# MarbleHE/ABC

Hardware: AMD Instinct MI355X
Metric: homomorphic mul+relin/sec, CKKS N=2^14 (higher is better)
Workload: dtype u64 (transforms: exact integer arithmetic in f64); 1 GPU; CKKS N=16384, 4 data limbs {50,40,40,40} + special 50-bit prime, ct x ct multiply + relinearize; total_batch=8192, batch_rank0=8192

## Files before the change

abc_amd/csrc/abc_context.hip:

```cpp
#include <cstdlib>
#include <cstring>
#include <mutex>

#include "../../include/abc_hip.h"
#include <dlfcn.h>

#include "abc_context.hpp"
#include "abc_host_math.hpp"

namespace abc {

static thread_local std::string g_err;
void set_error(const std::string &msg) { g_err = msg; }

static bool env_on(const char *name) {
  const char *e = std::getenv(name);
  return e && !(e[0] == '0' && e[1] == 0);
}
void read_switches(abc_hip_ctx *c) {
  abc_hip_ctx::Switches s;
  s.no_fused = env_on("ABC_HIP_NO_FUSED");
  s.no_split = env_on("ABC_HIP_NO_SPLIT");
  s.no_split4 = env_on("ABC_HIP_NO_SPLIT4");
  s.no_isplit = env_on("ABC_HIP_NO_ISPLIT");
  s.no_gsplit = env_on("ABC_HIP_NO_GSPLIT");
  s.no_bsplit = env_on("ABC_HIP_NO_BSPLIT");
  s.no_mixed = env_on("ABC_HIP_NO_MIXED");
  s.no_pack = env_on("ABC_HIP_NO_PACK");
  s.no_key_twin = env_on("ABC_HIP_NO_KEY_TWIN");
  s.no_bmul = env_on("ABC_HIP_NO_BMUL");
  s.no_iks = env_on("ABC_HIP_NO_IKS");
  s.no_lean_front = env_on("ABC_HIP_NO_LEAN_FRONT");
  s.no_tensor_intt = env_on("ABC_HIP_NO_TENSOR_INTT");
  s.no_galois_fusion = env_on("ABC_HIP_NO_GALOIS_FUSION");
  if (const char *e = std::getenv("ABC_HIP_CHUNK")) s.chunk = (size_t)std::atol(e);
  if (const char *e = std::getenv("ABC_HIP_FEW_LIMBS")) s.few_limbs = (size_t)std::atol(e);
  if (const char *e = std::getenv("ABC_HIP_LEAN_LIMIT")) s.lean_limit = (size_t)std::atol(e);
  if (const char *e = std::getenv("ABC_HIP_PASS0_TARGET_LIMIT")) s.pass0_target_limit = (size_t)std::atol(e);
  if (const char *e = std::getenv("ABC_HIP_BFV_SCRATCH_MB")) s.bfv_scratch_mb = (size_t)std::atol(e);
  if (const char *e = std::getenv("ABC_HIP_LANES")) {
    s.lanes = std::atoi(e);
    if (s.lanes < 1) s.lanes = 1;
    if (s.lanes > abc_hip_ctx::kMaxLanes) s.lanes = abc_hip_ctx::kMaxLanes;
  }
  c->sw = s;
}

static bool capturing(abc_hip_ctx *c) {
  hipStreamCaptureStatus st = hipStreamCaptureStatusNone;
  if (hipStreamIsCapturing(c->stream, &st) != hipSuccess) return false;
  return st != hipStreamCaptureStatusNone;
}

static int trim_cache(abc_hip_ctx *c) {
  std::lock_guard<std::mutex> lock(c->alloc_mu);
  if (c->free_blocks.empty()) return 0;
  ABC_HIP_CHECK(hipStreamSynchronize(c->stream));
  for (auto &kv : c->free_blocks)
    for (void *p : kv.second) {
      c->block_size.erase(p);
      (void)hipFree(p);
    }
  c->free_blocks.clear();
  c->cached_bytes = 0;
  return 0;
}
static hipError_t malloc_retry(abc_hip_ctx *c, void **p, size_t bytes) {
  hipError_t e = hipMalloc(p, bytes);
  if (e == hipSuccess) return e;
  (void)hipGetLastError();
  if (trim_cache(c)) return e;
  return hipMalloc(p, bytes);
}

void retire_buffer(abc_hip_ctx *c, void *p, uint64_t born) {
  if (!p) return;
  abc_hip_ctx::Held h{p, {}};
  for (auto &kv : c->live_graphs)
    if (kv.second > born) h.graphs.push_back(kv.first);
  if (h.graphs.empty()) {
    (void)hipFree(p);
    return;
  }
  c->held.push_back(std::move(h));
}

int ensure_workspace(abc_hip_ctx *c, size_t bytes) {
// ... 481 lines not shown
  }
}

int abc_hip_create_primes(size_t n, const int *bit_sizes, int count, uint64_t *out) {
  try {
    std::map<int, std::vector<uint64_t>> table;
    for (int i = 0; i < count; i++) table[bit_sizes[i]];
    for (auto &kv : table) {
      size_t need = 0;
      for (int i = 0; i < count; i++) need += (bit_sizes[i] == kv.first);
      kv.second = host::ntt_primes(n, kv.first, need);
    }
    for (int i = 0; i < count; i++) {
      auto &v = table[bit_sizes[i]];
      out[i] = v.back();
      v.pop_back();
    }
    return 0;
  } catch (const std::exception &e) {
    set_error(e.what());
    return 1;
  }
}

int abc_hip_ctx_create(int scheme, int logn, const uint64_t *primes, int nprimes, uint64_t plain_modulus, int device,
                       abc_hip_ctx **out) {
  if (!out) { set_error("null output pointer"); return 1; }
  *out = nullptr;
  if (scheme != ABC_HIP_SCHEME_BFV && scheme != ABC_HIP_SCHEME_CKKS) { set_error("unknown scheme"); return 1; }
  if (logn < 10 || logn > 16) { set_error("logn must be in 10..16"); return 1; }
  if (nprimes < 2 || nprimes > kMaxLimbs) { set_error("need 2..16 primes (data limbs + special prime)"); return 1; }
  const uint64_t two_n = 2ull << logn;
  for (int i = 0; i < nprimes; i++) {
    if (primes[i] >> 60 || !host::is_prime(primes[i]) || primes[i] % two_n != 1) {
      set_error("coefficient modulus primes must be < 2^60, prime and = 1 mod 2N");
      return 1;
    }
    for (int j = 0; j < i; j++)
      if (primes[j] == primes[i]) { set_error("coefficient modulus primes must be distinct"); return 1; }
  }
  if (scheme == ABC_HIP_SCHEME_BFV) {
    if (!host::is_prime(plain_modulus) || plain_modulus % two_n != 1 || plain_modulus >> 32) {
      set_error("plain modulus must be a prime = 1 mod 2N (batching) below 2^32");
      return 1;
    }
  }
  int ndev = 0;
  if (hipGetDeviceCount(&ndev) != hipSuccess || ndev <= 0) { set_error("no HIP device available"); return 1; }
  if (device < 0 || device >= ndev) { set_error("device index out of range"); return 1; }
  if (hipSetDevice(device) != hipSuccess) { set_error("hipSetDevice failed"); return 1; }
  abc_hip_ctx *c = new abc_hip_ctx();
  c->scheme = scheme; c->logn = logn; c->n = 1 << logn; c->K = nprimes; c->L = nprimes - 1; c->device = device;
  c->primes.assign(primes, primes + nprimes);
  c->t = (scheme == ABC_HIP_SCHEME_BFV) ? plain_modulus : 0;
  int rc = 1;
  try {
    rc = build_context(c);
  } catch (const std::exception &e) {
    set_error(e.what());
  }
  if (!rc && hipStreamCreateWithFlags(&c->own_stream, hipStreamNonBlocking) != hipSuccess) {
    set_error("hipStreamCreate failed");
    rc = 1;
  }
  if (!rc) c->stream = c->own_stream;
  if (!rc && (hipEventCreate(&c->ev0) != hipSuccess || hipEventCreate(&c->ev1) != hipSuccess ||
              hipEventCreateWithFlags(&c->lane_fork, hipEventDisableTiming) != hipSuccess)) {
    set_error("hipEventCreate failed");
    rc = 1;
  }
  for (int i = 0; !rc && i < abc_hip_ctx::kMaxLanes; i++) {
    if (hipStreamCreateWithFlags(&c->lane[i], hipStreamNonBlocking) != hipSuccess ||
        hipEventCreateWithFlags(&c->lane_join[i], hipEventDisableTiming) != hipSuccess) {
      set_error("lane stream / event creation failed");
      rc = 1;
    }
  }
  if (!rc && !env_on("ABC_HIP_SYNC_ALLOC")) {
    c->cache_alloc = true;
    size_t free_b = 0, total_b = 0;
    if (hipMemGetInfo(&free_b, &total_b) == hipSuccess) c->cache_cap = total_b / 4;
  }
  if (rc) { abc_hip_ctx_destroy(c); return 1; }
  *out = c;
  return 0;
}

void abc_hip_ctx_destroy(abc_hip_ctx *c) {
  if (!c) return;
  (void)hipSetDevice(c->device);
  (void)hipDeviceSynchronize();
  (void)hipFree(c->d_mods); (void)hipFree(c->d_tw); (void)hipFree(c->d_ftw); (void)hipFree(c->d_cst); (void)hipFree(c->d_cstf);
  (void)hipFree(c->d_slot_map);
  (void)hipFree(c->d_ckks_codec);
  drop_key_twins(c, nullptr);
  (void)hipFree(c->d_sk); (void)hipFree(c->d_pk); (void)hipFree(c->d_relin);
  for (auto &kv : c->d_galois) (void)hipFree(kv.second);
  (void)hipFree(c->ws);
  for (void *p : c->aux) (void)hipFree(p);
  for (auto &h : c->held) (void)hipFree(h.p);
  for (auto &kv : c->block_size) (void)hipFree(kv.first);
  if (c->own_stream) (void)hipStreamDestroy(c->own_stream);
  if (c->ev0) (void)hipEventDestroy(c->ev0);
  if (c->ev1) (void)hipEventDestroy(c->ev1);
  if (c->lane_fork) (void)hipEventDestroy(c->lane_fork);
  for (int i = 0; i < abc_hip_ctx::kMaxLanes; i++) {
// ... 487 lines not shown
```

abc_amd/csrc/abc_context.hpp:

```cpp
#pragma once

#include <hip/hip_runtime.h>

#include <map>
#include <mutex>
#include <unordered_map>
#include <string>
#include <vector>

#include "abc_modarith.hpp"
#include "abc_ntt.hpp"

namespace abc {

constexpr int kMaxLimbs = 16;

struct LimbMap {
  int id[kMaxLimbs + 1];
};

struct DevConst {
  u64 inv_special[kMaxLimbs], inv_special_s[kMaxLimbs];
  u64 inv_qlast[kMaxLimbs][kMaxLimbs], inv_qlast_s[kMaxLimbs][kMaxLimbs];
  u64 special_mod_q[kMaxLimbs], special_mod_q_s[kMaxLimbs];
// ... 24 lines not shown
  u64 tgamma_mod_q[kMaxLimbs], q_to_t[kMaxLimbs], q_to_gamma[kMaxLimbs];
  u64 neg_inv_q_mod_t, neg_inv_q_mod_gamma, inv_gamma_mod_t, gamma;
};

struct DevConstFp {
  double ext_q[kMaxLimbs][2], flr_q[kMaxLimbs][2], B_mod_q[kMaxLimbs][2];
  double q_to_bsk[kMaxLimbs][kMaxLimbs][2];
  double B_to_q[kMaxLimbs][kMaxLimbs][2];
  double q_mod_bsk[kMaxLimbs][2], inv_mtilde_mod_bsk[kMaxLimbs][2], tinvq_bsk[kMaxLimbs][2], inv_q_mod_bsk[kMaxLimbs][2];
  double inv_punct_B[kMaxLimbs][2], B_to_msk[kMaxLimbs][2], inv_B_mod_msk[2];
};

struct DevCtx {
  const Mod *mods;
  const u64 *tw;
  const double *ftw;
  const DevConst *cst;
  const DevConstFp *cstf;
  const u32 *slot_map;
  int logn, n;
  int ps;
  int K, L;
  int id_bsk, id_t, id_gamma, id_mtilde;
};

__device__ __forceinline__ NttTable ntt_table(const DevCtx &c, int mid) {
  const u64 *b = c.tw + (size_t)mid * 4 * c.n;
  NttTable t;
  t.tw = reinterpret_cast<const u64x2 *>(b);
  t.itw = reinterpret_cast<const u64x2 *>(b + 2 * (size_t)c.n);
  return t;
}

__device__ __forceinline__ Mod mod_at(const DevCtx &c, int id) {
  const ABC_CONST_AS Mod *p = (const ABC_CONST_AS Mod *)(c.mods + id);
  Mod m;
  m.q = p->q; m.mu = p->mu; m.two_q = p->two_q; m.shift = p->shift; m.bits = p->bits;
  m.inv_n = p->inv_n; m.inv_n_s = p->inv_n_s; m.qd = p->qd; m.qinv = p->qinv;
  m.inv_n_c = p->inv_n_c; m.inv_n_cq = p->inv_n_cq;
  return m;
}
__device__ __forceinline__ FpTable fp_table(const DevCtx &c, int mid) {
  const double *b = c.ftw + (size_t)mid * 4 * c.n;
  FpTable t;
  t.tw = (const ABC_CONST_AS f64x2 *)(b);
  t.itw = (const ABC_CONST_AS f64x2 *)(b + 2 * (size_t)c.n);
  return t;
}

}

struct abc_hip_ctx {
  int scheme = 0, logn = 0, n = 0, K = 0, L = 0, device = 0;
  std::vector<uint64_t> primes;
  uint64_t t = 0;
  hipStream_t stream = nullptr;
  hipStream_t own_stream = nullptr;
  hipEvent_t ev0 = nullptr, ev1 = nullptr;
  static constexpr int kMaxLanes = 4;
  hipStream_t lane[kMaxLanes] = {nullptr, nullptr, nullptr, nullptr};
  hipEvent_t lane_fork = nullptr, lane_join[kMaxLanes] = {nullptr, nullptr, nullptr, nullptr};
  std::vector<abc::Mod> h_mods;
  std::vector<uint64_t> mod_values;
  int nB = 0, nBsk = 0;
  abc::DevCtx dc{};
  abc::DevConst h_cst{};
  abc::Mod *d_mods = nullptr;
  uint64_t *d_tw = nullptr;
  double *d_ftw = nullptr;
  bool cache_alloc = false;
  std::mutex alloc_mu;
  size_t cached_bytes = 0, cache_cap = (size_t)8 << 30;
  std::unordered_map<size_t, std::vector<void *>> free_blocks;
  std::unordered_map<void *, size_t> block_size;
  bool capture_active = false;
  std::unordered_map<void *, std::vector<void *>> pin;
  std::unordered_map<void *, bool> parked;
  std::unordered_map<size_t, std::vector<void *>> cap_free;
  std::unordered_map<void *, bool> cap_born;
  bool behz_fp = false;
  bool use_fp = true;
  struct Switches {
    bool no_fused = false, no_split = false, no_split4 = false, no_isplit = false, no_gsplit = false, no_lean_front = false, no_bsplit = false, no_mixed = false, no_pack = false, no_key_twin = false, no_bmul = false, no_iks = false, no_tensor_intt = false;
    bool no_galois_fusion = false;
    size_t chunk = 0, few_limbs = 48, lean_limit = 96, bfv_scratch_mb = 0, pass0_target_limit = 128;
    int lanes = 2;
  } sw;
  abc::DevConst *d_cst = nullptr;
  abc::DevConstFp *d_cstf = nullptr;
  uint32_t *d_slot_map = nullptr;
  void *d_ckks_codec = nullptr;
  uint64_t *d_sk = nullptr, *d_pk = nullptr, *d_relin = nullptr;
  std::map<uint32_t, uint64_t *> d_galois;
  std::unordered_map<const uint64_t *, double *> key_twins;
  std::unordered_map<const uint64_t *, uint64_t *> key_shoups;
  std::vector<uint32_t> galois_order;
  void *ws = nullptr;
  size_t ws_bytes = 0;
  void *aux[3] = {nullptr, nullptr, nullptr};
  size_t aux_bytes[3] = {0, 0, 0};
  uint64_t graph_seq = 0;
  std::unordered_map<void *, uint64_t> live_graphs;
  struct Held {
    void *p;
    std::vector<void *> graphs;
  };
  std::vector<Held> held;
  uint64_t ws_born = 0, aux_born[3] = {0, 0, 0};
  size_t limb_words() const { return (size_t)n; }
  size_t key_words() const { return (size_t)L * 2 * K * n; }
};

namespace abc {

void set_error(const std::string &msg);
#define ABC_HIP_CHECK(expr)                                                                         \
  do {                                                                                              \
    hipError_t e_ = (expr);                                                                         \
    if (e_ != hipSuccess) {                                                                         \
      abc::set_error(std::string(#expr) + ": " + hipGetErrorString(e_));                            \
      return 1;                                                                                     \
    }                                                                                               \
  } while (0)

int ensure_workspace(abc_hip_ctx *c, size_t bytes);
int ensure_aux(abc_hip_ctx *c, int which, size_t bytes);
void retire_buffer(abc_hip_ctx *c, void *p, uint64_t born);
void read_switches(abc_hip_ctx *c);

LimbMap key_limb_map(const abc_hip_ctx *c, int nl);
int launch_ntt_fwd(abc_hip_ctx *c, u64 *d, const LimbMap &map, int nl, size_t total_limbs);
int launch_ks_expand_ntt_fp(abc_hip_ctx *c, const u64 *tcoef, size_t tstride, u64 *dec, const LimbMap &map, int nl, size_t count);
int launch_ntt_fwd_from2(abc_hip_ctx *c, const u64 *src, const u64 *src2, u64 *d, const LimbMap &map, int nl, size_t total_limbs);
int launch_ntt_fwd_from(abc_hip_ctx *c, const u64 *src, u64 *d, const LimbMap &map, int nl, size_t total_limbs);
int launch_ntt_inv(abc_hip_ctx *c, u64 *d, const LimbMap &map, int nl, size_t total_limbs);
int launch_ntt_inv_strided_part(abc_hip_ctx *c, u64 *d, const LimbMap &map, int nl, size_t total_limbs, bool integer_only = false);
int big_block_log(void);
// ... 146 lines not shown
```

abc_amd/csrc/abc_kernels_fused.hip:

```cpp
#include <type_traits>

#include "abc_context.hpp"
#include "abc_host_math.hpp"

namespace abc {

static inline unsigned stream_grid(size_t items, int block) {
  size_t g = (items + block - 1) / block;
  const size_t cap = 256 * 8 * 4;
  return (unsigned)(g < cap ? (g ? g : 1) : cap);
}

template <int LB>
__global__ __launch_bounds__((1 << LB) / 16) void k_fused_tensor_intt(DevCtx c, const u64 *__restrict__ a,
                                                                      const u64 *__restrict__ b, u64 *__restrict__ c01,
                                                                      u64 *__restrict__ c2coef, u64 *__restrict__ c2ntt, int nl) {
  __shared__ u64 lds[lds_words(LB)];
  const int j = blockIdx.x % nl;
  const size_t ct = blockIdx.x / nl;
  const size_t N = (size_t)1 << LB, pw = (size_t)nl * N;
  const Mod m = c.mods[j];
  const NttTable t = ntt_table(c, j);
  const u64 *__restrict__ a0 = a + ct * 2 * pw + j * N, *__restrict__ a1 = a0 + pw;
  const u64 *__restrict__ b0 = b + ct * 2 * pw + j * N, *__restrict__ b1 = b0 + pw;
// ... 416 lines not shown
        [&](int, int i, double v) {
          const double d = fp_mul_lazy(v, m.inv_n_c, m.inv_n_cq, m.qd) - (fp_from_u64(src[i]) + fix);
          o[i] = fp_to_canon(fp_mul_lazy(d, inv, inv_q, m.qd) + fp_from_u64(cin[i]), m.qd, m.qinv);
        },
        t, m, 0, 0);
  } else {
    ntt_inv_block_a<LB, FpArith>(
        lds, ld,
        [&](int, int i, double v) {
          const double d = fp_mul_lazy(v, m.inv_n_c, m.inv_n_cq, m.qd) - (fp_from_u64(src[i]) + fix);
          o[i] = fp_to_canon(fp_mul_lazy(d, inv, inv_q, m.qd), m.qd, m.qinv);
        },
        t, m, 0, 0);
  }
}

template <int LB>
__global__ __launch_bounds__((1 << LB) / 16) void k_fused_tensor_decomp_fp(DevCtx c, const u64 *__restrict__ a,
                                                                           const u64 *__restrict__ b, u64 *__restrict__ c01,
                                                                           u64 *__restrict__ c2ntt, u64 *__restrict__ dec, int nl) {
  __shared__ double lds[lds_words(LB)];
  const int j = blockIdx.x % nl;
  const size_t ct = blockIdx.x / nl;
  const size_t N = (size_t)1 << LB;
  double src[16];
  {
    const Mod m = mod_at(c, j);
    const FpTable t = fp_table(c, j);
    TensorFront front(a, b, c01, c2ntt, ct, j, nl, N, m);
    ntt_inv_block_a<LB, FpArith>(
        lds, [&](int r, int i) { return front(r, i); },
        [&](int r, int, double v) {
          const double w = fp_centre(fp_mul_lazy(v, m.inv_n_c, m.inv_n_cq, m.qd), m.qd, m.qinv);
          src[r] = w < 0.0 ? w + m.qd : w;
        },
        t, m, 0, 0);
  }
  for (int I = 0; I <= nl; I++) {
    if (I == j) continue;
    const int ki = (I == nl) ? c.K - 1 : I;
    const Mod m = mod_at(c, ki);
    const FpTable t = fp_table(c, ki);
    u64 *__restrict__ dst = dec + ((ct * (nl + 1) + I) * nl + j) * N;
    block_sync_lds();
    ntt_fwd_block_a<LB, FpArith>(
        lds, [&](int r, int) { return src[r]; }, [&](int, int i, double v) { dst[i] = fp_to_lazy(v, m.qd, m.qinv); }, t, m, 0, 0);
  }
}

template <int LB>
__device__ __forceinline__ void store_half_done(double *__restrict__ dst, double (&y)[16], int p, const FpK &kk, int kind) {
  constexpr size_t N = (size_t)1 << LB;
  constexpr int SH = LB - 4;
  if (kind == 0) {
#pragma unroll
    for (int k = 0; k < 16; k++) dst[(k << SH) + p] = y[k];
  } else if (kind == 1) {
#pragma unroll
    for (int k = 0; k < 16; k++) pack_store<1>(dst, N, (size_t)(k << SH) + p, fp_centre(y[k], kk.q, kk.qinv));
  } else {
#pragma unroll
    for (int k = 0; k < 16; k++) pack_store<2>(dst, N, (size_t)(k << SH) + p, fp_centre(y[k], kk.q, kk.qinv));
  }
}


template <int LB, bool CKKS, bool GAL>
__global__ __launch_bounds__((1 << LB) / 16) void k_fused_operand_pass0_fp(DevCtx c, const u64 *__restrict__ src, size_t src_stride,
                                                                           double *__restrict__ part, int nl, int per_target,
                                                                           u32 gelt, int padded) {
  static_assert(LB == 14, "split transforms are laid out for N = 2^14");
  __shared__ double lds[CKKS ? lds_words(LB) : 1];
  const size_t N = (size_t)1 << LB;
  const unsigned wg = per_target ? blockIdx.x / (unsigned)(nl + 1) : blockIdx.x;
  const int only = per_target ? (int)(blockIdx.x % (unsigned)(nl + 1)) : -1;
  const int j = wg % nl;
  const size_t ct = wg / nl;
  const int tid = threadIdx.x;
  const u64 *__restrict__ sp = src + ct * src_stride + (size_t)j * N;
  double x[16];
  if constexpr (CKKS) {
    const Mod m = mod_at(c, j);
    const FpTable t = fp_table(c, j);
    ntt_inv_block_a<LB, FpArith>(
        lds, [&](int, int i) { return fp_from_u64(sp[galois_ntt_src<GAL>((u32)i, gelt, LB)]); },
        [&](int r, int, double v) {
          double w = fp_centre(fp_mul_lazy(v, m.inv_n_c, m.inv_n_cq, m.qd), m.qd, m.qinv);
          x[r] = w < 0.0 ? w + m.qd : w;
        },
        t, m, 0, 0);
  } else if (gelt) {
    const u64 qj = c.mods[j].q;
#pragma unroll
    for (int k = 0; k < 16; k++) {
      bool neg;
      const u64 v = sp[galois_coef_src((u32)((k << 10) + tid), gelt, LB, neg)];
      x[k] = fp_from_u64(neg ? neg_mod(v, qj) : v);
    }
  } else {
#pragma unroll
    for (int k = 0; k < 16; k++) x[k] = fp_from_u64(sp[(k << 10) + tid]);
  }
  const int hi0[1] = {0};
  for (int I = 0; I <= nl; I++) {
    if (CKKS && I == j) continue;
    if (only >= 0 && I != only) continue;
    const int ki = (I == nl) ? c.K - 1 : I;
    const Mod m = mod_at(c, ki);
    const FpTable t = fp_table(c, ki);
    const FpK kk = FpArith::consts(m);
    double y[16];
#pragma unroll
    for (int k = 0; k < 16; k++) y[k] = x[k];
    fwd_pass<FpArith, LB, 0, 4>(y, hi0, t, kk, 0, 0);
    double *__restrict__ dst = part + ((ct * (nl + 1) + I) * nl + j) * ((padded & 1) ? (size_t)c.ps : N);
    store_half_done<LB>(dst, y, tid, kk, ((padded & 2) && I < nl) ? pack_kind(m.bits) : 0);
  }
}

template <int LB>
__global__ __launch_bounds__((1 << LB) / 16) void k_split2_tensor_pass0_fp(DevCtx c, const u64 *__restrict__ a,
                                                                           const u64 *__restrict__ b, double *__restrict__ part,
                                                                           int nl, int pack) {
  static_assert(LB == 14, "split transforms are laid out for N = 2^14");
  __shared__ double lds[lds_words(LB)];
  const int j = blockIdx.x % nl;
  const size_t ct = blockIdx.x / nl;
  const size_t N = (size_t)1 << LB, pw = (size_t)nl * N;
  double src[16];
  {
    const Mod m = mod_at(c, j);
    const FpTable t = fp_table(c, j);
    const u64 *__restrict__ a1 = a + ct * 2 * pw + pw + (size_t)j * N, *__restrict__ b1 = b + ct * 2 * pw + pw + (size_t)j * N;
    const double q = m.qd, qinv = m.qinv;
    ntt_inv_block_a<LB, FpArith>(
        lds, [&](int, int i) { return fp_mulmod(fp_from_u64(a1[i]), fp_from_u64(b1[i]), q, qinv); },
        [&](int r, int, double v) {
          const double w = fp_centre(fp_mul_lazy(v, m.inv_n_c, m.inv_n_cq, m.qd), m.qd, m.qinv);
          src[r] = w < 0.0 ? w + m.qd : w;
        },
        t, m, 0, 0);
  }
  const int tid = threadIdx.x;
  const int hi0[1] = {0};
  for (int I = 0; I <= nl; I++) {
    if (I == j) continue;
    const int ki = (I == nl) ? c.K - 1 : I;
    const Mod m = mod_at(c, ki);
    const FpTable t = fp_table(c, ki);
    const FpK kk = FpArith::consts(m);
    double y[16];
#pragma unroll
    for (int k = 0; k < 16; k++) y[k] = src[k];
    fwd_pass<FpArith, LB, 0, 4>(y, hi0, t, kk, 0, 0);
    double *__restrict__ dst = part + ((ct * (nl + 1) + I) * nl + j) * (size_t)c.ps;
    store_half_done<LB>(dst, y, tid, kk, (pack && I < nl) ? pack_kind(m.bits) : 0);
  }
}

template <int NL>
__global__ __launch_bounds__(NL ? NL * 64 : 768) void k_split_special_fp(DevCtx c, const double *__restrict__ part, const u64 *__restrict__ key,
                                                                         const double *__restrict__ keyf, double *__restrict__ tsp_half,
                                                                         int nl_rt) {
  extern __shared__ double dyn[];
  const int nl = NL ? NL : nl_rt;
  const int J = __builtin_amdgcn_readfirstlane((int)(threadIdx.x >> 6));
  const int lane = threadIdx.x & 63;
  const int blk = blockIdx.x & 15;
  const size_t ct = (size_t)(blockIdx.x >> 4);
  const size_t N = (size_t)c.n, base = (size_t)blk << 10;
  const int ki = c.K - 1;
  const Mod m = mod_at(c, ki);
  const FpTable t = fp_table(c, ki);
  const double q = m.qd, qinv = m.qinv;
  {
    double *buf = dyn + J * lds_words(10);
    const double *__restrict__ src = part + ((ct * (nl + 1) + nl) * nl + J) * (size_t)c.ps + base;
    ntt_fwd_block_a<10, FpTail>(
        buf, [&](int, int i) { return fp_centre(src[i], q, qinv); }, [&](int, int i, double v) { buf[lds_pad(i)] = v; }, t, m, 4, blk,
        lane);
  }
  __syncthreads();
  for (int e = 2 * (int)threadIdx.x; e < 1024; e += 2 * (int)blockDim.x) {
    double s0[2] = {0.0, 0.0}, s1[2] = {0.0, 0.0};
#pragma unroll
    for (int Jx = 0; Jx < (NL ? NL : 12); Jx++) {
      if (!NL && Jx >= nl) break;
      const f64x2 v = *reinterpret_cast<const f64x2 *>(dyn + Jx * lds_words(10) + lds_pad(e));
      const size_t i0 = (((size_t)Jx * 2 + 0) * c.K + ki) * N + base + e, i1 = i0 + (size_t)c.K * N;
      f64x2 k0, k1;
      if (keyf) {
        k0 = *reinterpret_cast<const f64x2 *>(keyf + i0);
        k1 = *reinterpret_cast<const f64x2 *>(keyf + i1);
      } else {
        const u64x2 r0 = *reinterpret_cast<const u64x2 *>(key + i0), r1 = *reinterpret_cast<const u64x2 *>(key + i1);
        k0.x = fp_from_u64(r0.x); k0.y = fp_from_u64(r0.y);
        k1.x = fp_from_u64(r1.x); k1.y = fp_from_u64(r1.y);
      }
      s0[0] += fp_mulmod(v.x, k0.x, q, qinv);
      s0[1] += fp_mulmod(v.y, k0.y, q, qinv);
      s1[0] += fp_mulmod(v.x, k1.x, q, qinv);
      s1[1] += fp_mulmod(v.y, k1.y, q, qinv);
      if (Jx == 7) {
#pragma unroll
        for (int k = 0; k < 2; k++) {
          s0[k] = fp_centre(s0[k], q, qinv);
          s1[k] = fp_centre(s1[k], q, qinv);
        }
      }
    }
// ... 497 lines not shown
  return 0;
}
int join_lanes(abc_hip_ctx *c, int lanes) {
  if (lanes < 2) return 0;
  for (int l = 0; l < lanes; l++) {
    ABC_HIP_CHECK(hipEventRecord(c->lane_join[l], c->lane[l]));
    ABC_HIP_CHECK(hipStreamWaitEvent(c->stream, c->lane_join[l], 0));
  }
  return 0;
}

static int run_isplit(abc_hip_ctx *c, int mode, const u64 *opa, const u64 *opb, size_t opa_stride, size_t opb_stride, bool add_c1,
                      const u64 *key, u64 *out, int nl, size_t count, u32 gelt) {
  const size_t N = (size_t)c->n;
  const ChunkPlan p = plan_chunks(c, nl, count);
  const bool twin = c->logn == 14 && !c->sw.no_mixed;
  return for_each_chunk(c, count, p.chunk, p.lanes, isplit_scratch_words(c, nl), twin ? key : nullptr,
                        [&](hipStream_t st, u64 *scratch, size_t off, size_t cc) {
                          return isplit_chunk(c, st, scratch, cc, nl, mode, opa + off * opa_stride, opb ? opb + off * opb_stride : nullptr,
                                              opa_stride, opb_stride, add_c1 ? 1 : 0, key, out + off * 2 * (size_t)nl * N, gelt);
                        });
}

static int run_gsplit15(abc_hip_ctx *c, int mode, const u64 *opa, const u64 *opb, size_t opa_stride, size_t opb_stride, bool add_c1,
                        const u64 *key, u64 *out, int nl, size_t count, u32 gelt) {
  const size_t N = (size_t)c->n;
  const ChunkPlan p = plan_chunks(c, nl, count);
  return for_each_chunk(c, count, p.chunk, p.lanes, gsplit_scratch_words(c, nl), nullptr,
                        [&](hipStream_t st, u64 *scratch, size_t off, size_t cc) {
                          return gsplit_chunk15(c, st, scratch, cc, nl, mode, opa + off * opa_stride, opb ? opb + off * opb_stride : nullptr,
                                                opa_stride, opb_stride, add_c1 ? 1 : 0, key, out + off * 2 * (size_t)nl * N, gelt);
                        });
}

template <int LB>
static int run_mul_relin(abc_hip_ctx *c, const u64 *a, const u64 *b, u64 *out, int nl, size_t count) {
  const size_t N = (size_t)1 << LB;
  if (LB == 14 && !all_fp(c) && isplit_applies(c, nl))
    return run_isplit(c, 0, a, b, 2 * (size_t)nl * N, 2 * (size_t)nl * N, false, c->d_relin, out, nl, count, 0u);
  const ChunkPlan p = plan_chunks(c, nl, count);
  const bool split = LB == 14 && all_fp(c) && !c->sw.no_split && nl <= 12;
  const size_t SN = split ? (size_t)c->dc.ps : N;
  const size_t per_ct = fused_scratch_limbs(nl) * SN;
  const size_t ctw = 2 * (size_t)nl * N;
  return for_each_chunk(c, count, p.chunk, p.lanes, per_ct, split ? c->d_relin : nullptr, [&](hipStream_t st, u64 *scratch, size_t off, size_t cc) {
    const FusedScratch s = carve(scratch, p.chunk, nl, SN);
    if constexpr (LB == 14) {
      if (split) {
        const bool lean = !c->sw.no_lean_front && cc * nl <= c->sw.lean_limit;
        const int pack = pack_half_done(c, nl);
        if (lean)
          gsplit_front14(st, c, cc, nl, 0, a + off * ctw, b + off * ctw, 0, (double *)s.coef, (double *)s.dec, 0u, pack);
        else
          hipLaunchKernelGGL(k_split2_tensor_pass0_fp<LB>, dim3((unsigned)(cc * nl)), dim3((1 << LB) / 16), 0, st, c->dc, a + off * ctw,
                             b + off * ctw, (double *)s.dec, nl, pack);
        launch_split3<0, false>(st, c, s, cc, nl, a + off * ctw, b + off * ctw, 0, 0, 0, c->d_relin, out + off * ctw, 0u, pack);
        ABC_HIP_CHECK(hipGetLastError());
        return 0;
      }
    }
    if (all_fp(c))
      hipLaunchKernelGGL(k_fused_tensor_decomp_fp<LB>, dim3((unsigned)(cc * nl)), dim3((1 << LB) / 16), 0, st, c->dc, a + off * ctw,
                         b + off * ctw, s.c01, s.ntt, s.dec, nl);
    else
      hipLaunchKernelGGL(k_fused_tensor_intt<LB>, dim3((unsigned)(cc * nl)), dim3((1 << LB) / 16), 0, st, c->dc, a + off * ctw,
                         b + off * ctw, s.c01, s.coef, s.ntt, nl);
    return keyswitch_stage<LB>(c, st, s, s.coef, (size_t)nl * N, s.ntt, (size_t)nl * N, c->d_relin, s.c01, ctw, true, out + off * ctw, nl,
                               cc, all_fp(c) ? 1 : 0);
  });
}

int ckks_mul_relin_fused(abc_hip_ctx *c, const u64 *a, const u64 *b, u64 *out, int nl, size_t count) {
  if (c->logn == 15 && gsplit_applies(c, nl)) {
    if (!count) return 0;
    const size_t ctw = 2 * (size_t)nl * c->n;
    return run_gsplit15(c, 0, a, b, ctw, ctw, false, c->d_relin, out, nl, count, 0u);
  }
  if (c->logn == 15 && !all_fp(c) && isplit_applies(c, nl)) {
    if (!count) return 0;
    const size_t ctw = 2 * (size_t)nl * c->n;
    return run_isplit(c, 0, a, b, ctw, ctw, false, c->d_relin, out, nl, count, 0u);
  }
  if (c->logn > 14) return -1;
  if (c->sw.no_fused) return -1;
  if (!count) return 0;
  switch (c->logn) {
    case 10: return run_mul_relin<10>(c, a, b, out, nl, count);
    case 11: return run_mul_relin<11>(c, a, b, out, nl, count);
    case 12: return run_mul_relin<12>(c, a, b, out, nl, count);
    case 13: return run_mul_relin<13>(c, a, b, out, nl, count);
    case 14: return run_mul_relin<14>(c, a, b, out, nl, count);
    default: return -1;
  }
}

template <int LB>
static int run_keyswitch(abc_hip_ctx *c, const u64 *target, size_t target_stride, const u64 *key, u64 *out, int nl, size_t count,
                         const u64 *addend, size_t addend_stride, bool add_c1, u32 gelt = 0) {
  const size_t N = (size_t)1 << LB;
  const bool ckks = (c->scheme == 2);
  if (LB == 14 && ckks && !all_fp(c) && isplit_applies(c, nl))
    return run_isplit(c, 1, target, addend, target_stride, addend_stride, add_c1, key, out, nl, count, gelt);
  const ChunkPlan p = plan_chunks(c, nl, count);
  const bool splitc = LB == 14 && ckks && all_fp(c) && !c->sw.no_split && nl <= 12;
  const bool splitb = LB == 14 && !ckks && !c->sw.no_split && bsplit_applies(c, nl);
  const u32 ginv = (!ckks && gelt) ? (u32)host::invmod(gelt, 2 * (uint64_t)N) : 0u;
  if (ginv && !splitb) { set_error("run_keyswitch: a BFV permutation is only folded into the split sequence"); return 1; }
  const size_t SN = (splitc || splitb) ? (size_t)c->dc.ps : N;
// ... 109 lines not shown
```

abc_amd/csrc/abc_ntt.hpp:

```cpp
#pragma once

#include "abc_modarith.hpp"

namespace abc {

__device__ __forceinline__ int lds_pad(int i) { return i + ((i >> 6) << 2); }
constexpr int lds_words(int lb) { return (1 << lb) + ((1 << lb) >> 6) * 4; }

struct NttTable {
  const u64x2 *tw;
  const u64x2 *itw;
};
struct alignas(16) f64x2 {
  double x, y;
};
#define ABC_CONST_AS __attribute__((address_space(4)))
struct FpTable {
  const ABC_CONST_AS f64x2 *tw, *itw;
};
__device__ __forceinline__ f64x2 tw_load(const ABC_CONST_AS f64x2 *p) {
  f64x2 r;
  r.x = p->x;
  r.y = p->y;
  return r;
}
__device__ __forceinline__ u64x2 tw_load(const u64x2 *p) { return *p; }

struct FpK {
  double q, qinv;
  bool red;
};
#pragma clang fp contract(off)
__device__ __forceinline__ double fp_mul_lazy(double y, double w, double wq, double q) {
  const double h = y * w;
  const double l = __builtin_fma(y, w, -h);
  const double c = __builtin_rint(y * wq);
  return __builtin_fma(-c, q, h) + l;
}
__device__ __forceinline__ double fp_centre(double x, double q, double qinv) {
  return __builtin_fma(-__builtin_rint(x * qinv), q, x);
}
__device__ __forceinline__ double fp_from_u64(u64 v) {
  return __longlong_as_double((long long)(v | 0x4330000000000000ull)) - 4503599627370496.0;
}
__device__ __forceinline__ u64 fp_to_canon(double x, double q, double qinv) {
  double r = fp_centre(x, q, qinv);
  const u32 neg = (u32)((int)(u32)((u64)__double_as_longlong(r) >> 32) >> 31);
  const u64 qb = (u64)__double_as_longlong(q);
  const u64 add = ((u64)((u32)(qb >> 32) & neg) << 32) | (u64)((u32)qb & neg);
  r += __longlong_as_double((long long)add);
  return (u64)__double_as_longlong(r + 4503599627370496.0) & 0x000fffffffffffffull;
}
__device__ __forceinline__ u64 fp_to_lazy(double x, double q, double qinv) {
  const double r = fp_centre(x, q, qinv);
  return (u64)__double_as_longlong(r + (4503599627370496.0 + q)) & 0x000fffffffffffffull;
}
__host__ __device__ __forceinline__ bool fp_ok(u32 bits) { return bits <= 50; }

__host__ __device__ __forceinline__ int pack_kind(u32 bits) { return bits <= 40 ? 1 : bits <= 48 ? 2 : 0; }
constexpr double kPackMagic = 6755399441055744.0;
template <int PK>
__device__ __forceinline__ void pack_store(double *limb, size_t n, size_t idx, double centred) {
  const u64 b = (u64)__double_as_longlong(centred + kPackMagic);
  reinterpret_cast<u32 *>(limb)[idx] = (u32)b;
  if (PK == 1) reinterpret_cast<unsigned char *>(limb)[4 * n + idx] = (unsigned char)(b >> 32);
  else reinterpret_cast<unsigned short *>(reinterpret_cast<unsigned char *>(limb) + 4 * n)[idx] = (unsigned short)(b >> 32);
}
template <int PK>
__device__ __forceinline__ u64x2 pack_load_pair(const double *limb, size_t n, size_t idx) {
  u64x2 r;
  r.x = *reinterpret_cast<const u64 *>(reinterpret_cast<const u32 *>(limb) + idx);
  if (PK == 1) r.y = *reinterpret_cast<const unsigned short *>(reinterpret_cast<const unsigned char *>(limb) + 4 * n + idx);
  else r.y = *reinterpret_cast<const u32 *>(reinterpret_cast<const unsigned char *>(limb) + 4 * n + 2 * idx);
  return r;
}
template <int PK>
__device__ __forceinline__ void pack_decode_pair(const u64x2 &r, double &v0, double &v1) {
  const u32 h = (u32)r.y;
  const int h0 = PK == 1 ? (int)(signed char)(h & 0xffu) : (int)(short)(h & 0xffffu);
  const int h1 = PK == 1 ? (int)(signed char)((h >> 8) & 0xffu) : ((int)h >> 16);
  const u64 b0 = ((u64)(u32)(0x43380000 + h0) << 32) | (u32)r.x;
  const u64 b1 = ((u64)(u32)(0x43380000 + h1) << 32) | (u32)(r.x >> 32);
  v0 = __longlong_as_double((long long)b0) - kPackMagic;
  v1 = __longlong_as_double((long long)b1) - kPackMagic;
}

template <bool GUARD>
struct IntArith {
  using E = u64;
  using TW = u64x2;
  using Table = NttTable;
  struct K {
    u64 q, two_q;
  };
  __device__ __forceinline__ static K consts(const Mod &m) { return K{m.q, m.two_q}; }
  __device__ __forceinline__ static void fwd(E &X, E &Y, const TW tp, const K &k) {
    if (GUARD) {
      const u64 a = csub(X, k.two_q);
      const u64 v = mul_shoup_lazy(Y, tp.x, tp.y, k.q);
      X = a + v;
      Y = a + k.two_q - v;
    } else {
      const u64 a = X;
      const u64 v = mul_shoup_lazy4(Y, tp.x, tp.y, k.q);
      X = a + v;
      Y = a + (k.two_q << 1) - v;
    }
  }
  __device__ __forceinline__ static void inv(E &X, E &Y, const TW tp, const K &k) {
    const u64 a = X, c = Y;
    X = csub(a + c, k.two_q);
    Y = mul_shoup_lazy(a + k.two_q - c, tp.x, tp.y, k.q);
  }
  template <int PASS> __device__ __forceinline__ static void fwd_begin(E (&)[16], const K &) {}
  template <int PASS> __device__ __forceinline__ static void inv_begin(E (&)[16], const K &) {}
};

struct FpArith {
  using E = double;
// ... 439 lines not shown
```

Baseline: 400,600 mul+relin/s.

## Make tensor pass0 a persistent task loop with prefetch of next slice

The split tensor pass0 kernel becomes persistent, with one block per CU looping over (ciphertext, limb) tasks. While each task runs its forward NTT stores, the block prefetches the next task's input slices with inline-asm global loads and stages their products into LDS, so load latency overlaps the store phase. The stores also switch to wave-uniform scalar base plus lane offset addressing to cut address VGPR work. The cost is heavier register pressure, fragile hand-written vmcnt waits, and fewer resident blocks if the grid is capped at the CU count.

```diff
diff --git a/abc_amd/csrc/abc_context.hip b/abc_amd/csrc/abc_context.hip
--- a/abc_amd/csrc/abc_context.hip
+++ b/abc_amd/csrc/abc_context.hip
@@ -33,6 +33,7 @@
   s.no_lean_front = env_on("ABC_HIP_NO_LEAN_FRONT");
   s.no_tensor_intt = env_on("ABC_HIP_NO_TENSOR_INTT");
   s.no_galois_fusion = env_on("ABC_HIP_NO_GALOIS_FUSION");
+  s.no_task_loop = env_on("ABC_HIP_NO_TASK_LOOP");
   if (const char *e = std::getenv("ABC_HIP_CHUNK")) s.chunk = (size_t)std::atol(e);
   if (const char *e = std::getenv("ABC_HIP_FEW_LIMBS")) s.few_limbs = (size_t)std::atol(e);
   if (const char *e = std::getenv("ABC_HIP_LEAN_LIMIT")) s.lean_limit = (size_t)std::atol(e);
@@ -620,6 +621,7 @@
   abc_hip_ctx *c = new abc_hip_ctx();
   c->scheme = scheme; c->logn = logn; c->n = 1 << logn; c->K = nprimes; c->L = nprimes - 1; c->device = device;
   c->primes.assign(primes, primes + nprimes);
+  if (hipDeviceGetAttribute(&c->cus, hipDeviceAttributeMultiprocessorCount, device) != hipSuccess) c->cus = 0;
   c->t = (scheme == ABC_HIP_SCHEME_BFV) ? plain_modulus : 0;
   int rc = 1;
   try {
diff --git a/abc_amd/csrc/abc_context.hpp b/abc_amd/csrc/abc_context.hpp
--- a/abc_amd/csrc/abc_context.hpp
+++ b/abc_amd/csrc/abc_context.hpp
@@ -100,6 +100,7 @@
 
 struct abc_hip_ctx {
   int scheme = 0, logn = 0, n = 0, K = 0, L = 0, device = 0;
+  int cus = 0;
   std::vector<uint64_t> primes;
   uint64_t t = 0;
   hipStream_t stream = nullptr;
@@ -130,7 +131,7 @@
   bool use_fp = true;
   struct Switches {
     bool no_fused = false, no_split = false, no_split4 = false, no_isplit = false, no_gsplit = false, no_lean_front = false, no_bsplit = false, no_mixed = false, no_pack = false, no_key_twin = false, no_bmul = false, no_iks = false, no_tensor_intt = false;
-    bool no_galois_fusion = false;
+    bool no_galois_fusion = false, no_task_loop = false;
     size_t chunk = 0, few_limbs = 48, lean_limit = 96, bfv_scratch_mb = 0, pass0_target_limit = 128;
     int lanes = 2;
   } sw;
diff --git a/abc_amd/csrc/abc_kernels_fused.hip b/abc_amd/csrc/abc_kernels_fused.hip
--- a/abc_amd/csrc/abc_kernels_fused.hip
+++ b/abc_amd/csrc/abc_kernels_fused.hip
@@ -492,15 +492,32 @@
 __device__ __forceinline__ void store_half_done(double *__restrict__ dst, double (&y)[16], int p, const FpK &kk, int kind) {
   constexpr size_t N = (size_t)1 << LB;
   constexpr int SH = LB - 4;
+  const gbyte *base = wave_uniform_base(dst);
+  const u32 lane4 = (u32)p << 2;
   if (kind == 0) {
-#pragma unroll
-    for (int k = 0; k < 16; k++) dst[(k << SH) + p] = y[k];
-  } else if (kind == 1) {
-#pragma unroll
-    for (int k = 0; k < 16; k++) pack_store<1>(dst, N, (size_t)(k << SH) + p, fp_centre(y[k], kk.q, kk.qinv));
+    const u32 l8 = lane_offset_here(lane4 << 1);
+#pragma unroll
+    for (int k = 0; k < 16; k++)
+      *reinterpret_cast<__attribute__((address_space(1))) double *>(wave_uniform_base(base + ((size_t)k << (SH + 3))) + l8) = y[k];
   } else {
-#pragma unroll
-    for (int k = 0; k < 16; k++) pack_store<2>(dst, N, (size_t)(k << SH) + p, fp_centre(y[k], kk.q, kk.qinv));
+    const int hs = kind - 1;
+    const u32 laneh = (lane4 >> 2) << hs;
+#pragma unroll
+    for (int k0 = 0; k0 < 16; k0 += 4) {
+      u32 hw[4];
+      const u32 l4 = lane_offset_here(lane4), lh = lane_offset_here(laneh);
+#pragma unroll
+      for (int k = 0; k < 4; k++) hw[k] = pack_store_low(wave_uniform_base(base + ((size_t)(k0 + k) << (SH + 2))), l4, fp_centre(y[k0 + k], kk.q, kk.qinv));
+      if (kind == 1) {
+#pragma unroll
+        for (int k = 0; k < 4; k++) *(wave_uniform_base(base + 4 * N + ((size_t)(k0 + k) << SH)) + lane_offset_here(lh)) = (unsigned char)hw[k];
+      } else {
+#pragma unroll
+        for (int k = 0; k < 4; k++)
+          *reinterpret_cast<__attribute__((address_space(1))) unsigned short *>(wave_uniform_base(base + 4 * N + ((size_t)(k0 + k) << (SH + 1))) + lane_offset_here(lh)) =
+              (unsigned short)hw[k];
+      }
+    }
   }
 }
 
@@ -561,41 +578,134 @@
 template <int LB>
 __global__ __launch_bounds__((1 << LB) / 16) void k_split2_tensor_pass0_fp(DevCtx c, const u64 *__restrict__ a,
                                                                            const u64 *__restrict__ b, double *__restrict__ part,
-                                                                           int nl, int pack) {
+                                                                           int nl, int pack, unsigned ntasks) {
   static_assert(LB == 14, "split transforms are laid out for N = 2^14");
   __shared__ double lds[lds_words(LB)];
-  const int j = blockIdx.x % nl;
-  const size_t ct = blockIdx.x / nl;
+  using P0 = PassIdx<LB, LB - Sched<LB>::R3, Sched<LB>::R3>;
+  static_assert(P0::NG == 4 && P0::G == 1, "the staging below is written for four groups of four adjacent elements");
   const size_t N = (size_t)1 << LB, pw = (size_t)nl * N;
-  double src[16];
-  {
-    const Mod m = mod_at(c, j);
-    const FpTable t = fp_table(c, j);
-    const u64 *__restrict__ a1 = a + ct * 2 * pw + pw + (size_t)j * N, *__restrict__ b1 = b + ct * 2 * pw + pw + (size_t)j * N;
-    const double q = m.qd, qinv = m.qinv;
-    ntt_inv_block_a<LB, FpArith>(
-        lds, [&](int, int i) { return fp_mulmod(fp_from_u64(a1[i]), fp_from_u64(b1[i]), q, qinv); },
-        [&](int r, int, double v) {
-          const double w = fp_centre(fp_mul_lazy(v, m.inv_n_c, m.inv_n_cq, m.qd), m.qd, m.qinv);
-          src[r] = w < 0.0 ? w + m.qd : w;
-        },
-        t, m, 0, 0);
-  }
   const int tid = threadIdx.x;
   const int hi0[1] = {0};
-  for (int I = 0; I <= nl; I++) {
-    if (I == j) continue;
-    const int ki = (I == nl) ? c.K - 1 : I;
-    const Mod m = mod_at(c, ki);
-    const FpTable t = fp_table(c, ki);
-    const FpK kk = FpArith::consts(m);
-    double y[16];
-#pragma unroll
-    for (int k = 0; k < 16; k++) y[k] = src[k];
-    fwd_pass<FpArith, LB, 0, 4>(y, hi0, t, kk, 0, 0);
-    double *__restrict__ dst = part + ((ct * (nl + 1) + I) * nl + j) * (size_t)c.ps;
-    store_half_done<LB>(dst, y, tid, kk, (pack && I < nl) ? pack_kind(m.bits) : 0);
-  }
+  const int e0 = 4 * (__builtin_amdgcn_readfirstlane(tid >> 6) * 256 + (tid & 63));
+  struct Slice {
+    u32x4 a[2], b[2];
+  };
+  const auto slice_load = [&](const gbyte *a1, const gbyte *b1, int g, u32 off) {
+    Slice v;
+    const gbyte *pa = wave_uniform_base(a1 + 2048 * g), *pb = wave_uniform_base(b1 + 2048 * g);
+    asm volatile(
+        "global_load_dwordx4 %0, %4, %5\n\tglobal_load_dwordx4 %1, %4, %5 offset:16\n\t"
+        "global_load_dwordx4 %2, %4, %6\n\tglobal_load_dwordx4 %3, %4, %6 offset:16"
+        : "=&v"(v.a[0]), "=&v"(v.a[1]), "=&v"(v.b[0]), "=&v"(v.b[1])
+        : "v"(off), "s"(pa), "s"(pb)
+        : "memory");
+    return v;
+  };
+  const auto slice_wait = [&](Slice &v, int stores) {
+    if (stores == 32) asm volatile("s_waitcnt vmcnt(32)" : "+v"(v.a[0]), "+v"(v.a[1]), "+v"(v.b[0]), "+v"(v.b[1]) : : "memory");
+    else if (stores == 16) asm volatile("s_waitcnt vmcnt(16)" : "+v"(v.a[0]), "+v"(v.a[1]), "+v"(v.b[0]), "+v"(v.b[1]) : : "memory");
+    else asm volatile("s_waitcnt vmcnt(0)" : "+v"(v.a[0]), "+v"(v.a[1]), "+v"(v.b[0]), "+v"(v.b[1]) : : "memory");
+  };
+  const auto dbl = [](u32 lo, u32 hi) { return fp_from_u64(((u64)hi << 32) | lo); };
+  const auto slice_stage = [&](const Slice &v, int g, double q, double qinv) {
+    double *w = lds + lds_pad(e0 + 256 * g);
+    w[0] = fp_mulmod(dbl(v.a[0].x, v.a[0].y), dbl(v.b[0].x, v.b[0].y), q, qinv);
+    w[1] = fp_mulmod(dbl(v.a[0].z, v.a[0].w), dbl(v.b[0].z, v.b[0].w), q, qinv);
+    w[2] = fp_mulmod(dbl(v.a[1].x, v.a[1].y), dbl(v.b[1].x, v.b[1].y), q, qinv);
+    w[3] = fp_mulmod(dbl(v.a[1].z, v.a[1].w), dbl(v.b[1].z, v.b[1].w), q, qinv);
+  };
+  bool staged = false;
+  for (unsigned task = blockIdx.x; task < ntasks; task += gridDim.x) {
+    const int j = __builtin_amdgcn_readfirstlane((int)(task % (unsigned)nl));
+    const size_t ct = (unsigned)__builtin_amdgcn_readfirstlane((int)(task / (unsigned)nl));
+    double src[16];
+    {
+      const Mod m = mod_at(c, j);
+      const FpTable t = fp_table(c, j);
+      double x0[16];
+      if (!staged) {
+        const u64 *__restrict__ a1 = a + ct * 2 * pw + pw + (size_t)j * N, *__restrict__ b1 = b + ct * 2 * pw + pw + (size_t)j * N;
+        const double q = m.qd, qinv = m.qinv;
+#pragma unroll
+        for (int g = 0; g < 4; g++) {
+          const u64x2 *pa = reinterpret_cast<const u64x2 *>(a1 + e0 + 256 * g), *pb = reinterpret_cast<const u64x2 *>(b1 + e0 + 256 * g);
+#pragma unroll
+          for (int h = 0; h < 2; h++) {
+            const u64x2 va = pa[h], vb = pb[h];
+            x0[4 * g + 2 * h] = fp_mulmod(fp_from_u64(va.x), fp_from_u64(vb.x), q, qinv);
+            x0[4 * g + 2 * h + 1] = fp_mulmod(fp_from_u64(va.y), fp_from_u64(vb.y), q, qinv);
+          }
+        }
+      } else {
+#pragma unroll
+        for (int r = 0; r < 16; r++) x0[r] = lds[lds_pad(e0 + 256 * (r >> 2)) + (r & 3)];
+      }
+      ntt_inv_block_a<LB, FpArith>(
+          lds, [&](int r, int) { return x0[r]; },
+          [&](int r, int, double v) {
+            const double w = fp_centre(fp_mul_lazy(v, m.inv_n_c, m.inv_n_cq, m.qd), m.qd, m.qinv);
+            src[r] = w < 0.0 ? w + m.qd : w;
+          },
+          t, m, 0, 0);
+    }
+    const unsigned next = task + gridDim.x;
+    const bool more = next < ntasks;
+    const int jn = __builtin_amdgcn_readfirstlane((int)(next % (unsigned)nl));
+    const size_t ctn = (unsigned)__builtin_amdgcn_readfirstlane((int)(next / (unsigned)nl));
+    const gbyte *an1 = wave_uniform_base(a + ctn * 2 * pw + pw + (size_t)jn * N), *bn1 = wave_uniform_base(b + ctn * 2 * pw + pw + (size_t)jn * N);
+    double qn = 0.0, qninv = 0.0;
+    if (more) {
+      const Mod mn = mod_at(c, jn);
+      qn = mn.qd;
+      qninv = mn.qinv;
+      block_sync_lds();
+    }
+    const auto forward = [&](int I, auto stage_tag, int g) {
+      constexpr bool STAGE = decltype(stage_tag)::value;
+      const int ki = (I == nl) ? c.K - 1 : I;
+      const Mod m = mod_at(c, ki);
+      const FpTable t = fp_table(c, ki);
+      const FpK kk = FpArith::consts(m);
+      double y[16];
+#pragma unroll
+      for (int k = 0; k < 16; k++) y[k] = src[k];
+      fwd_pass<FpArith, LB, 0, 4>(y, hi0, t, kk, 0, 0);
+      Slice v;
+      if constexpr (STAGE) {
+        u32 off = (u32)e0 << 3;
+        asm volatile("" : "+v"(off) : "v"(y[0]), "v"(y[1]), "v"(y[2]), "v"(y[3]), "v"(y[4]), "v"(y[5]), "v"(y[6]), "v"(y[7]), "v"(y[8]),
+                       "v"(y[9]), "v"(y[10]), "v"(y[11]), "v"(y[12]), "v"(y[13]), "v"(y[14]), "v"(y[15]));
+        v = slice_load(an1, bn1, g, off);
+      }
+      double *__restrict__ dst = part + ((ct * (nl + 1) + I) * nl + j) * (size_t)c.ps;
+      const int kind = (pack && I < nl) ? pack_kind(m.bits) : 0;
+      store_half_done<LB>(dst, y, tid, kk, kind);
+      if constexpr (STAGE) {
+        slice_wait(v, kind ? 32 : 16);
+        slice_stage(v, g, qn, qninv);
+      }
+    };
+    int I = 0, g = 0;
+    if (more) {
+      for (; I <= nl && g < 4; I++)
+        if (I != j) forward(I, std::true_type{}, g++);
+    }
+    for (; I <= nl; I++)
+      if (I != j) forward(I, std::false_type{}, 0);
+    for (; more && g < 4; g++) {
+      Slice v = slice_load(an1, bn1, g, lane_offset_here((u32)e0 << 3));
+      slice_wait(v, 0);
+      slice_stage(v, g, qn, qninv);
+    }
+    staged = more;
+  }
+}
+
+template <int LB>
+static void launch_tensor_pass0(hipStream_t st, abc_hip_ctx *c, size_t cc, int nl, const u64 *a, const u64 *b, double *part, int pack) {
+  const unsigned tasks = (unsigned)(cc * nl);
+  const unsigned grid = (c->sw.no_task_loop || c->cus <= 0 || tasks < (unsigned)c->cus) ? tasks : (unsigned)c->cus;
+  hipLaunchKernelGGL(k_split2_tensor_pass0_fp<LB>, dim3(grid), dim3((1 << LB) / 16), 0, st, c->dc, a, b, part, nl, pack, tasks);
 }
 
 template <int NL>
@@ -1199,8 +1309,7 @@
         if (lean)
           gsplit_front14(st, c, cc, nl, 0, a + off * ctw, b + off * ctw, 0, (double *)s.coef, (double *)s.dec, 0u, pack);
         else
-          hipLaunchKernelGGL(k_split2_tensor_pass0_fp<LB>, dim3((unsigned)(cc * nl)), dim3((1 << LB) / 16), 0, st, c->dc, a + off * ctw,
-                             b + off * ctw, (double *)s.dec, nl, pack);
+          launch_tensor_pass0<LB>(st, c, cc, nl, a + off * ctw, b + off * ctw, (double *)s.dec, pack);
         launch_split3<0, false>(st, c, s, cc, nl, a + off * ctw, b + off * ctw, 0, 0, 0, c->d_relin, out + off * ctw, 0u, pack);
         ABC_HIP_CHECK(hipGetLastError());
         return 0;
diff --git a/abc_amd/csrc/abc_ntt.hpp b/abc_amd/csrc/abc_ntt.hpp
--- a/abc_amd/csrc/abc_ntt.hpp
+++ b/abc_amd/csrc/abc_ntt.hpp
@@ -65,6 +65,23 @@
   reinterpret_cast<u32 *>(limb)[idx] = (u32)b;
   if (PK == 1) reinterpret_cast<unsigned char *>(limb)[4 * n + idx] = (unsigned char)(b >> 32);
   else reinterpret_cast<unsigned short *>(reinterpret_cast<unsigned char *>(limb) + 4 * n)[idx] = (unsigned short)(b >> 32);
+}
+typedef __attribute__((address_space(1))) unsigned char gbyte;
+typedef u32 u32x4 __attribute__((ext_vector_type(4)));
+template <class T>
+__device__ __forceinline__ gbyte *wave_uniform_base(const T *p) {
+  const u64 v = (u64)p;
+  const u32 lo = (u32)__builtin_amdgcn_readfirstlane((int)(u32)v), hi = (u32)__builtin_amdgcn_readfirstlane((int)(u32)(v >> 32));
+  return (gbyte *)(((u64)hi << 32) | lo);
+}
+__device__ __forceinline__ u32 lane_offset_here(u32 v) {
+  asm volatile("" : "+v"(v));
+  return v;
+}
+__device__ __forceinline__ u32 pack_store_low(gbyte *lo, u32 lane4, double centred) {
+  const u64 b = (u64)__double_as_longlong(centred + kPackMagic);
+  *reinterpret_cast<__attribute__((address_space(1))) u32 *>(lo + lane4) = (u32)b;
+  return (u32)(b >> 32);
 }
 template <int PK>
 __device__ __forceinline__ u64x2 pack_load_pair(const double *limb, size_t n, size_t idx) {
```

Result: no change. 399,900 mul+relin/s (median of 2 runs) (-0.2%).
